# second-state/qwen3_asr_rs

Hardware: AMD Instinct MI355X
Metric: audio-seconds/sec (RTFx) Qwen3-ASR-0.6B greedy, 30s clips (higher is better)
Workload: dtype bf16; 1 GPU; Qwen3-ASR-0.6b bf16, batch=1 x 30s synthetic 16kHz clip per GPU, 100 new tokens (fixed, EOS ignored); clips_per_gpu=1, parallelism=dp1 (independent utterances per GPU, no data-path collective)

## Files before the change

qwen3_asr_rs_amd/csrc/engine.cpp:

```cpp
#include <hip/hip_runtime.h>

#include <sched.h>

#include <chrono>
#include <cmath>
#include <cstdio>
#include <cstring>
#include <map>
#include <memory>
#include <mutex>
#include <thread>

#include "engine_internal.h"

using namespace q3a;

namespace {

thread_local std::string g_last_error;

constexpr int kGemvMaxSeq = 2;

template <typename T>
void upload(DevBuf& b, const std::vector<T>& v, hipStream_t s) {
// ... 73 lines not shown
  const std::vector<hipEvent_t>& join_ev; const hipEvent_t& fork_ev; const int& n_cu; int* const& host_prog_dev;
  std::vector<ProfEvent>* const& prof; Taps& taps;
  const int8_t* const& lm_q; const float* const& lm_qs; const int& lm_q_cols;
  const int &B, &max_ctx, &max_new, &gsize, &live_nsplit_, &attn_nsplit, &min_P_, &part_stride, &beam_w_;
  const size_t& kv_layer_elems; const bool& head_logits_;
  const int &k_parallel_groups, &k_skinny_q, &k_dattn_batched_min_wgs, &k_skinny_glu_hp3, &k_lm_head_prune;
  const bool& logit_bias_on_;
  const bool& sampling_on_;
  const bool& repetition_on_;

  bool precise() const { return opts.precise != 0; }
  bool token_lp() const { return opts.token_logprobs != 0; }
  bool kv_f32() const { return opts.precise != 0; }
  size_t kv_elem() const { return kv_f32() ? 4 : 2; }
  int fast_math() const { return precise() ? 0 : 1; }
  template <typename T> const T* w(uint64_t off) const { return reinterpret_cast<const T*>(arena + off); }
  const float* wf(uint64_t off) const { return w<float>(off); }
  const uint16_t* wh(uint64_t off) const { return w<uint16_t>(off); }
};

struct DecodeStep : StepView {
  DevBuf kcache, vcache, x_dec, d_pos, next_tok, out_ids, step_count, done, s_ln, s_qkv, s_ctx, s_act, logits, part_val, part_idx;
  DevBuf part_sum, out_lp;
  DevBuf blk_lo, blk_hi;
  DevBuf prune_stats;
  DevBuf attn_pm, attn_pl, attn_po, nn_x, nn_ss;
  DevBuf rope_cur, rope_cos, rope_sin;
  DevBuf n_done, forced_tok;
  DevBuf beam_cand_val, beam_cand_idx, beam_part_max, beam_part_sum, beam_topk_ids, beam_topk_lp, beam_score, beam_finished, beam_parent, beam_token;
  DevBuf beam_feed, beam_hist_parent, beam_hist_token, beam_hist_lp, beam_state, beam_lo;
  DevBuf logit_bias;
  DevBuf samp_params, samp_max, samp_sum;
  DevBuf rep_params;
  DevBuf draft_accepted;
  template <class Self, class F> static void each_buf(Self& s, F&& f) {
    for (auto* b : {&s.kcache, &s.vcache, &s.x_dec, &s.d_pos, &s.next_tok, &s.out_ids, &s.step_count, &s.done, &s.s_ln, &s.s_qkv, &s.s_ctx, &s.s_act, &s.logits,
                    &s.part_val, &s.part_idx, &s.part_sum, &s.out_lp, &s.blk_lo, &s.blk_hi, &s.prune_stats, &s.attn_pm, &s.attn_pl, &s.attn_po, &s.nn_x, &s.nn_ss,
                    &s.rope_cur, &s.rope_cos, &s.rope_sin, &s.n_done, &s.forced_tok,
                    &s.beam_cand_val, &s.beam_cand_idx, &s.beam_part_max, &s.beam_part_sum, &s.beam_topk_ids, &s.beam_topk_lp, &s.beam_score, &s.beam_finished,
                    &s.beam_parent, &s.beam_token, &s.beam_feed, &s.beam_hist_parent, &s.beam_hist_token, &s.beam_hist_lp, &s.beam_state, &s.beam_lo,
                    &s.logit_bias, &s.samp_params, &s.samp_max, &s.samp_sum, &s.rep_params, &s.draft_accepted})
      f(*b);
  }

  void tap(const char* name, const void* ptr, size_t bytes) { taps.copy(opts.debug_taps, stream, name, ptr, bytes); }
  template <class F> void timed(int kclass, double bytes, F&& fn) {
    if (!prof) return fn();
    ProfEvent pe{kclass, bytes, nullptr, nullptr};
    HIPCHK(hipEventCreate(&pe.a));
    HIPCHK(hipEventCreate(&pe.b));
    HIPCHK(hipEventRecord(pe.a, stream));
    fn();
    HIPCHK(hipEventRecord(pe.b, stream));
    prof->push_back(pe);
  }

  void* kc_layer(int l) { return (uint8_t*)kcache.p + (size_t)l * kv_layer_elems * kv_elem(); }
  void* vc_layer(int l) { return (uint8_t*)vcache.p + (size_t)l * kv_layer_elems * kv_elem(); }

  LmHeadPruneArgs prune_args(const GemvArgs& g) {
    LmHeadPruneArgs pa{};
    pa.g = g; pa.Wq = lm_q; pa.qcols = lm_q_cols; pa.qs = lm_qs;
    pa.blk_lo = blk_lo.as<float>(); pa.blk_hi = blk_hi.as<float>(); pa.stats = prune_stats.as<int>();
    pa.logit_bias = g.bias != nullptr;
    return pa;
  }

  const float* head_bias() const { return logit_bias_on_ ? logit_bias.as<float>() : nullptr; }

  void run_head(int advance) {
    const int S = B, H = d.hidden, V = d.vocab;
    const float* const hb = head_bias();
    const bool sample = sampling_on_, repeat = repetition_on_, store = head_logits_ || sample || repeat;
    tap("head_in", x_dec.p, (size_t)S * H * 4);
    const double wbytes = 2.0 * V * H;
    int n_part = 0;
    const ArgmaxPartials part{part_val.as<float>(), part_idx.as<int>(), token_lp() ? part_sum.as<float>() : nullptr, part_stride};
    if (S <= kGemvMaxSeq) {
      GemvArgs g{};
      g.fast_math = fast_math();
      g.x = x_dec.as<float>(); g.ldx = H; g.rms_w = wf(L.final_norm); g.eps = d.rms_eps;
      g.W = wh(L.lm_head); g.N = V; g.K = H; g.mode = 3; g.out = logits.as<float>(); g.ldo = V;
      g.part = part; g.bias = hb;
      LmHeadPruneArgs pa{};
      const bool prunable = S == 1 && !precise() && lm_q_cols > 0 && (pa = prune_args(g), !lm_head_prune_check(pa));
      if (prunable && opts.debug_taps == 1) {
        DevBuf& t = taps.reserve("lm_head_bound", (size_t)V * 8);
        LmHeadPruneArgs pd = pa;
        pd.dbg = t.as<float>(); pd.stats = nullptr;
        KCHK(launch_lm_head_approx(pd, stream));
      }
      if (prunable && k_lm_head_prune && !store) {
        g.out = nullptr; pa.g.out = nullptr;
        n_part = lm_head_rescore_groups(g, n_cu);
        timed(Q3A_KC_GEMV_LM_HEAD, (double)V * lm_q_cols, [&] { KCHK(launch_lm_head_approx(pa, stream)); });
        timed(Q3A_KC_ARGMAX, 0, [&] { KCHK(launch_lm_head_rescore(pa, n_part, stream)); });
      } else {
        n_part = gemv_blocks(g);
        timed(Q3A_KC_GEMV_LM_HEAD, wbytes, [&] { KCHK(launch_gemv(g, S, stream)); });
      }
    } else if (!precise()) {
      timed(Q3A_KC_NORM, 0, [&] { KCHK(launch_rmsnorm(x_dec.as<float>(), wf(L.final_norm), s_ln.as<float>(), S, H, d.rms_eps, stream, s_ln.as<uint16_t>())); });
      GemmEpilogue ep; ep.out = logits.as<float>(); ep.ldo = V; ep.bias = hb;
      if (S <= 32 && V % 4 == 0 && H % 64 == 0 && part_stride >= (V + 63) / 64) {
        ep.part = part;
        if (!store) ep.out = nullptr;
        n_part = (V + 63) / 64;
        timed(Q3A_KC_GEMM, wbytes, [&] { KCHK(launch_gemm16(s_ln.as<uint16_t>(), H, wh(L.lm_head), S, V, H, ep, false, stream)); });
      } else {
        timed(Q3A_KC_GEMM, wbytes, [&] { KCHK(launch_gemm16(s_ln.as<uint16_t>(), H, wh(L.lm_head), S, V, H, ep, false, stream)); });
        n_part = 128;
        if (!repeat) timed(Q3A_KC_ARGMAX, 0, [&] { KCHK(launch_argmax_partials(logits.as<float>(), V, S, part, n_part, stream)); });
      }
    } else {
      timed(Q3A_KC_NORM, 0, [&] { KCHK(launch_rmsnorm(x_dec.as<float>(), wf(L.final_norm), s_ln.as<float>(), S, H, d.rms_eps, stream)); });
      timed(Q3A_KC_GEMM, wbytes, [&] { batched_proj(s_ln.as<float>(), H, wh(L.lm_head), V, H, hb, 0, logits.as<float>(), V, nullptr); });
      n_part = 128;
      if (!repeat) timed(Q3A_KC_ARGMAX, 0, [&] { KCHK(launch_argmax_partials(logits.as<float>(), V, S, part, n_part, stream)); });
    }
    if (repeat) n_part = enqueue_repetition(part, !sample);
    FinalizeArgs f{};
    f.part = part; f.n_part = n_part; f.out_lp = part.sum ? out_lp.as<float>() : nullptr;
    f.V = V; f.next_tok = next_tok.as<int>(); f.out_ids = out_ids.as<int>();
    f.out_stride = max_new; f.step_count = step_count.as<int>(); f.pos = d_pos.as<int>(); f.advance = advance;
    f.done = done.as<uint8_t>(); f.n_done = n_done.as<int>(); f.n_seq = S; f.host_progress = host_prog_dev; f.embed = wh(L.embed); f.H = H; f.x_next = x_dec.as<float>(); f.eos0 = kEos0; f.eos1 = kEos1;
    f.cos_t = rope_cos.as<float>(); f.sin_t = rope_sin.as<float>(); f.rope_cur = rope_cur.as<float>();
    f.nn = first_layer_norm_out();
    if (sample) enqueue_sampler(f);
    timed(Q3A_KC_ARGMAX, 0, [&] { KCHK(launch_argmax_finalize(f, S, stream)); });
    if (sample && token_lp()) enqueue_sample_logprob();
  }
  void enqueue_draft_accept(DraftAcceptArgs a) {
    a.n_seq = B; a.accepted = draft_accepted.as<int>();
    a.next_tok = next_tok.as<int>(); a.out_ids = out_ids.as<int>(); a.out_stride = max_new; a.step_count = step_count.as<int>(); a.pos = d_pos.as<int>();
    a.out_lp = token_lp() ? out_lp.as<float>() : nullptr;
    a.done = done.as<uint8_t>(); a.n_done = n_done.as<int>(); a.host_progress = host_prog_dev;
    a.embed = wh(L.embed); a.H = d.hidden; a.x_next = x_dec.as<float>(); a.eos0 = kEos0; a.eos1 = kEos1;
    a.cos_t = rope_cos.as<float>(); a.sin_t = rope_sin.as<float>(); a.rope_cur = rope_cur.as<float>();
    a.nn = first_layer_norm_out();
    timed(Q3A_KC_ARGMAX, 0, [&] { KCHK(launch_draft_accept(a, stream)); });
  }
  int enqueue_repetition(const ArgmaxPartials& part, bool partials) {
    RepeatArgs ra{};
    ra.logits = logits.as<float>(); ra.S = B; ra.V = d.vocab; ra.params = rep_params.as<uint32_t>();
    ra.out_ids = out_ids.as<int>(); ra.out_stride = max_new; ra.step_count = step_count.as<int>();
    timed(Q3A_KC_ARGMAX, 0, [&] { KCHK(launch_repeat_apply(ra, stream)); });
    constexpr int kRepeatParts = 128;
    if (partials) timed(Q3A_KC_ARGMAX, 0, [&] { KCHK(launch_argmax_partials(ra.logits, ra.V, ra.S, part, kRepeatParts, stream)); });
    return kRepeatParts;
  }
// ... 330 lines not shown

  void init_common(const std::string& model_dir, int dev, const q3a_opts* o) {
    if (o) opts = *o; else q3a_opts_default(&opts);
    if (opts.max_new_tokens <= 0) opts.max_new_tokens = 4096;
    d = parse_config_file(model_dir + "/config.json");
    validate_dims(d);
    L = plan_arena(d);
    device = dev;
    int n_dev = 0;
    hipError_t e = hipGetDeviceCount(&n_dev);
    if (e != hipSuccess || n_dev == 0)
      fail("no HIP device available: libq3asr_hip has no CPU fallback (hipGetDeviceCount: " + std::string(hipGetErrorString(e)) + ")");
    if (dev < 0 || dev >= n_dev) fail("device index out of range");
    HIPCHK(hipSetDevice(dev));
    KCHK(skinny_init());
    (void)hipDeviceGetAttribute(&n_cu, hipDeviceAttributeMultiprocessorCount, dev);
    HIPCHK(hipStreamCreateWithFlags(&stream, hipStreamNonBlocking));
    for (auto& x : ev) HIPCHK(hipEventCreate(&x));
    HIPCHK(hipHostMalloc((void**)&host_prog, 64, hipHostMallocMapped));
    memset(host_prog, 0, 64);
    HIPCHK(hipHostGetDevicePointer((void**)&host_prog_dev, host_prog, 0));
    step.n_done.ensure(64);
    step.prune_stats.ensure(8);
    HIPCHK(hipMemsetAsync(step.prune_stats.p, 0, 8, stream));
    if (!d.aligner()) {
      step.logit_bias.ensure((size_t)d.vocab * 4);
      HIPCHK(hipMemsetAsync(step.logit_bias.p, 0, (size_t)d.vocab * 4, stream));
      logit_bias_finite_ = d.vocab;
      step.samp_params.ensure(16);
      step.rep_params.ensure(16);
    }
  }

  void init_tables() {
    auto dftm = make_dft_matrix(400, 416);
    auto filt = make_mel_filterbank_T(d.n_mels, 400, 16000, 202);
    auto pe = make_sinusoid_rows(d.tokens_per_chunk(), d.enc_d);
    upload(dft, dftm, stream);
    upload(filt_t, filt, stream);
    upload(pos_emb, pe, stream);
    zero_page.ensure(256);
    HIPCHK(hipMemsetAsync(zero_page.p, 0, 256, stream));
    ensure_rope(8192);
    HIPCHK(hipStreamSynchronize(stream));
  }

// ... 381 lines not shown
    kv_layer_elems = (size_t)b * d.n_kv * max_ctx * 128;
    step.kcache.ensure(kv_layer_elems * d.dec_layers * kv_elem());
    step.vcache.ensure(kv_layer_elems * d.dec_layers * kv_elem());
    step.rope_cur.ensure((size_t)b * 128 * 4);
    {
      Knobs& kn = knobs();
      const int gs = kn.decode_group_size.load();
      gsize = (gs >= 1 && gs <= 32) ? gs : 32;
      k_parallel_groups = kn.decode_parallel_groups.load(); k_skinny_q = kn.skinny_q.load();
      k_dattn_batched_min_wgs = kn.dattn_batched_min_wgs.load();
      k_skinny_glu_hp3 = kn.skinny_glu_hp3.load();
      k_lm_head_prune = kn.lm_head_prune.load();
    }
    const size_t ng = (size_t)step.n_groups(b);
    step.nn_x.ensure(ng * 32 * H * 2); step.nn_ss.ensure((size_t)ng * (H / 8) * 32 * 4);
    step.x_dec.ensure((size_t)b * H * 4); step.next_tok.ensure((size_t)b * 4); step.forced_tok.ensure((size_t)b * 4); step.draft_accepted.ensure((size_t)b * 8);
    step.out_ids.ensure((size_t)b * max_new * 4); step.step_count.ensure((size_t)b * 4); step.done.ensure((size_t)b);
    step.s_ln.ensure((size_t)b * H * 4); step.s_qkv.ensure((size_t)b * d.qkv_dim() * 4); step.s_ctx.ensure(ng * 32 * d.q_dim() * 4);
    step.s_act.ensure(ng * 32 * d.inter * 4); step.logits.ensure((size_t)b * d.vocab * 4);
    part_stride = std::max(128, (d.vocab + 3) / 4);
    step.part_val.ensure((size_t)b * part_stride * 4); step.part_idx.ensure((size_t)b * part_stride * 4);
    if (token_lp()) { step.part_sum.ensure((size_t)b * part_stride * 4); step.out_lp.ensure((size_t)b * max_new * 4); }
    if (sampling_on_) { step.samp_max.ensure((size_t)b * sample_chunks(d.vocab) * 4); step.samp_sum.ensure((size_t)b * sample_chunks(d.vocab) * 4); }
    {
      const size_t nblk4 = ((size_t)(d.vocab + 15) / 16 + 3) & ~size_t(3);
      step.blk_lo.ensure(nblk4 * 4); step.blk_hi.ensure(nblk4 * 4);
    }
    attn_nsplit = (max_ctx + dattn_keys_per_split(kv_f32()) - 1) / dattn_keys_per_split(kv_f32());
    {
      const size_t n_stat = (size_t)b * d.n_q * attn_nsplit;
      step.attn_pm.ensure((n_stat + 8) * 4); step.attn_pl.ensure((n_stat + 8) * 4);
      step.attn_po.ensure(n_stat * 128 * 4);
      if (knobs().poison_attn_partials.load() != 0) {
        HIPCHK(hipMemsetAsync(step.attn_pm.p, 0xFF, step.attn_pm.cap, stream));
        HIPCHK(hipMemsetAsync(step.attn_pl.p, 0xFF, step.attn_pl.cap, stream));
        HIPCHK(hipMemsetAsync(step.attn_po.p, 0xFF, step.attn_po.cap, stream));
      }
    }
    HIPCHK(hipMemsetAsync(step.step_count.p, 0, (size_t)b * 4, stream));
    HIPCHK(hipMemsetAsync(step.done.p, 0, (size_t)b, stream));
    HIPCHK(hipMemsetAsync(step.n_done.p, 0, 64, stream));
    HIPCHK(hipMemsetAsync(step.out_ids.p, 0, (size_t)b * max_new * 4, stream));
    if (token_lp()) HIPCHK(hipMemsetAsync(step.out_lp.p, 0, (size_t)b * max_new * 4, stream));
    HIPCHK(hipStreamSynchronize(stream));
    for (auto cs : chain_streams) HIPCHK(hipStreamSynchronize(cs));
    __atomic_store_n(&host_prog[0], 0, __ATOMIC_RELAXED);
    __atomic_store_n(&host_prog[1], 0, __ATOMIC_RELAXED);
    drain_retired_graphs();
    {
      bool any = false;
      DecodeStep::each_buf(step, [&](DevBuf& sb) { any = any || sb.grew; sb.grew = false; });
      if (any) drop_graphs();
    }
  }

  void run_prefill() {
    run_prefill_layers();
    const int H = d.hidden;
    KCHK(launch_gather_rows(dec_x.as<float>(), last_rows.as<int>(), B, H, step.x_dec.as<float>(), stream));
    tap("dec_last_hidden", step.x_dec.p, (size_t)B * H * 4);
    step.run_head(0);
    tap("logits", step.logits.p, (size_t)B * d.vocab * 4);
    HIPCHK(hipGetLastError());
    have_prefill = true;
// ... 1415 lines not shown
```

qwen3_asr_rs_amd/csrc/k_decode.hip:

```cpp
#include "argmax.h"
#include "embed_row.h"

namespace q3a {

namespace {

__global__ void embed_kernel(const int* __restrict__ ids, const uint16_t* __restrict__ embed, int H, int skip_id,
                             float* __restrict__ out) {
  const int r = blockIdx.x;
  const int id = ids[r];
  if (id == skip_id) return;
  const uint2* src = reinterpret_cast<const uint2*>(embed + (size_t)id * H);
  float4* dst = reinterpret_cast<float4*>(out + (size_t)r * H);
  for (int i = threadIdx.x; i < H / 4; i += blockDim.x) {
    const uint2 v = src[i];
    dst[i] = make_float4(bf16lo(v.x), bf16hi(v.x), bf16lo(v.y), bf16hi(v.y));
  }
}

__global__ void set_tokens_kernel(const int* __restrict__ tok, const uint16_t* __restrict__ embed, int H,
                                  float* __restrict__ x_next, int* __restrict__ next_tok, NextNormOut nn) {
  __shared__ float red[16];
  const int s = blockIdx.x;
  const int id = tok[s];
// ... 90 lines not shown
  for (int o = 32; o > 0; o >>= 1) m.merge_lane(o);
  if (lane == 0) {
    bv[wave] = m.v; bi[wave] = m.i;
    if constexpr (LP) bs[wave] = m.s;
  }
  __syncthreads();
  if (tid == 0) {
    for (int w = 1; w < 16; ++w) m.merge(bv[w], bi[w], bs[LP ? w : 0]);
    int idx = m.i;
    float lp = 0.f;
    if constexpr (LP) {
      lp = -logf(m.s);
      if (lp > 0.f) lp = 0.f;
    }
    if (idx < 0 || idx >= a.V) { idx = 0; lp = __int_as_float(0x7fc00000); }
    tok_s = idx;
    a.next_tok[s] = idx;
    if (sc < a.out_stride) a.out_ids[(size_t)s * a.out_stride + sc] = idx;
    if constexpr (LP) {
      if (sc < a.out_stride) a.out_lp[(size_t)s * a.out_stride + sc] = lp;
    }
    a.step_count[s] = sc + 1;
    a.pos[s] = np;
    if ((idx == a.eos0 || idx == a.eos1) && !was_done) {
      a.done[s] = 1;
      if (a.n_done) {
        const int n = atomicAdd(a.n_done, 1) + 1;
        if (n == a.n_seq && a.host_progress) __hip_atomic_store(a.host_progress + 1, 1, __ATOMIC_RELAXED, __HIP_MEMORY_SCOPE_SYSTEM);
      }
    }
    if (s == 0 && a.host_progress) __hip_atomic_store(a.host_progress, sc + 1, __ATOMIC_RELAXED, __HIP_MEMORY_SCOPE_SYSTEM);
  }
  __syncthreads();
  if (a.rope_cur && tid < 128) a.rope_cur[(size_t)s * 128 + tid] = rope_v;
  embed_row(a.embed, tok_s, a.H, a.x_next, s, a.nn, bv);
}

}

const char* launch_embed(const int* ids, int rows, const uint16_t* embed, int H, int skip_id, float* out,
                         hipStream_t s) {
  if (rows <= 0) return nullptr;
  hipLaunchKernelGGL(embed_kernel, dim3(rows), dim3(256), 0, s, ids, embed, H, skip_id, out);
  return nullptr;
}
const char* launch_set_tokens(const int* tok, int S, const uint16_t* embed, int H, float* x_next, int* next_tok,
// ... 33 lines not shown
```

qwen3_asr_rs_amd/csrc/k_gemv.hip:

```cpp
#include <algorithm>

#include "argmax.h"


namespace q3a {

int gemv_rows_per_wave(const GemvArgs& a) {
  const int logical = (a.mode == 2) ? a.N / 2 : a.N;
  static const int mid = [] { const char* e = getenv("Q3A_GEMV_PR_MID"); return e ? atoi(e) : 2; }();
  static const int small = [] { const char* e = getenv("Q3A_GEMV_PR_SMALL"); return e ? atoi(e) : 1; }();
  if (logical >= 32768 && a.K <= 2048) return 4;
  if (logical >= 4096 || a.mode == 2) return (mid == 4 || mid == 2) ? mid : 2;
  return (small == 1 || small == 2 || small == 4) ? small : 1;
}
int gemv_blocks(const GemvArgs& a) {
  const int pr = gemv_rows_per_wave(a);
  const int rows_per_wave = (a.mode == 2) ? pr / 2 : pr;
  const int logical = (a.mode == 2) ? a.N / 2 : a.N;
  return (logical + 4 * rows_per_wave - 1) / (4 * rows_per_wave);
}

namespace {

constexpr int ATTN_F_MAX = 1024;
// ... 369 lines not shown
  for (int it = 0; it < KI; ++it)
#pragma unroll
    for (int i = 0; i < PR; ++i) acc[i][0] = dot8(wq[it][i], x[it], acc[i][0]);
  if (wave == 0) asm volatile("" ::"v"(acc[0][0]));
  Q3A_STAMP_AT(a.stamp, blockIdx.x, 3);
  float rstd = 1.0f;
  if (RMS) rstd = rstd_of(wave_sum_fast(ss) / (float)K + a.eps, a.fast_math != 0);
#pragma unroll
  for (int i = 0; i < PR; ++i) acc[i][0] = wave_sum_fast(acc[i][0]) * rstd + bv[i];
  if (lane != 0) return;
  if (a.mode != 2) {
#pragma unroll
    for (int i = 0; i < PR; ++i)
      if (prow[i] >= 0) a.out[prow[i]] = acc[i][0] + rv[i];
  } else {
#pragma unroll
    for (int i = 0; i + 1 < PR; i += 2)
      if (prow[i] >= 0) a.out[g * (PR / 2) + (i >> 1)] = silu_sel(acc[i][0], a.fast_math != 0) * acc[i + 1][0];
  }
  Q3A_STAMP_AT(a.stamp, blockIdx.x, 4);
}

template <int PR, int KI, bool LP = false>
__device__ __forceinline__ void gemv1_head_block(const GemvArgs& a, int blk, float (&am_v)[4][1], int (&am_i)[4][1], float* am_s,
                                                 ArgmaxAcc<LP>& out) {
  const int tid = threadIdx.x, lane = tid & 63, wave = tid >> 6;
  const int K = a.K;
  const int g = blk * 4 + wave;
  int prow[PR];
  gemv_rows<PR>(a, g, prow);
  bool kin[KI];
  int kk[KI];
#pragma unroll
  for (int it = 0; it < KI; ++it) {
    const int k = lane * 8 + it * 512;
    kin[it] = k < K;
    kk[it] = kin[it] ? k : 0;
  }
  float4 xr[KI][2], nr[KI][2];
  uint4 wq[KI][PR];
#pragma unroll
  for (int it = 0; it < KI; ++it) {
    xr[it][0] = *reinterpret_cast<const float4*>(a.x + kk[it]);
    xr[it][1] = *reinterpret_cast<const float4*>(a.x + kk[it] + 4);
    nr[it][0] = *reinterpret_cast<const float4*>(a.rms_w + kk[it]);
    nr[it][1] = *reinterpret_cast<const float4*>(a.rms_w + kk[it] + 4);
  }
#pragma unroll
  for (int it = 0; it < KI; ++it)
#pragma unroll
    for (int i = 0; i < PR; ++i) {
// ... 14 lines not shown
    for (int e = 0; e < 8; ++e) x[it][e] = (K == KI * 512 || kin[it]) ? xv[e] : 0.f;
    const float4 w0 = nr[it][0], w1 = nr[it][1];
    const float wv[8] = {w0.x, w0.y, w0.z, w0.w, w1.x, w1.y, w1.z, w1.w};
#pragma unroll
    for (int e = 0; e < 8; ++e) { ss += x[it][e] * x[it][e]; x[it][e] *= wv[e]; }
  }
  float acc[PR];
#pragma unroll
  for (int i = 0; i < PR; ++i) acc[i] = 0.f;
#pragma unroll
  for (int it = 0; it < KI; ++it)
#pragma unroll
    for (int i = 0; i < PR; ++i) acc[i] = dot8(wq[it][i], x[it], acc[i]);
  const float rstd = rstd_of(wave_sum_fast(ss) / (float)K + a.eps, a.fast_math != 0);
#pragma unroll
  for (int i = 0; i < PR; ++i) acc[i] = wave_sum_fast(acc[i]) * rstd + bv[i];
  ArgmaxAcc<LP> m;
#pragma unroll
  for (int i = 0; i < PR; ++i) {
    if (prow[i] < 0) continue;
    if (lane == 0 && a.out) a.out[prow[i]] = acc[i];
    if (acc[i] > m.v) { m.v = acc[i]; m.i = prow[i]; }
  }
  if (lane == 0) { am_v[wave][0] = m.v; am_i[wave][0] = m.i; }
  if constexpr (LP) {
    float ws = 0.f;
#pragma unroll
    for (int i = 0; i < PR; ++i) ws += prow[i] < 0 ? 0.f : lse_term(1.f, acc[i], m.v);
    if (lane == 0) am_s[wave] = ws;
  }
  __syncthreads();
  if (tid == 0) {
    out = {am_v[0][0], am_i[0][0], LP ? am_s[0] : 0.f};
    for (int w = 1; w < 4; ++w) out.merge(am_v[w][0], am_i[w][0], LP ? am_s[w] : 0.f);
  }
}

template <int PR, int KI, bool LP = false>
__global__ __launch_bounds__(256) void gemv1_head_kernel(GemvArgs a) {
  __shared__ float am_v[4][1];
  __shared__ int am_i[4][1];
  __shared__ float am_s[LP ? 4 : 1];
  ArgmaxAcc<LP> r;
  gemv1_head_block<PR, KI, LP>(a, blockIdx.x, am_v, am_i, am_s, r);
  if (threadIdx.x == 0) r.store(a.part, 0, blockIdx.x);
}

struct LmHeadArgsDev {
  GemvArgs g;
  const int8_t* Wq; const float* qs; int qcols;
  float gamma;
  float* blk_lo; float* blk_hi; int n_blk;
  float* dbg;
  int* stats;
};

__device__ __forceinline__ float dotq8(uint32_t lo, uint32_t hi, const float (&x)[8], float s) {
  f32x2_t a = f32x2_t{(float)(int8_t)lo, (float)(int8_t)(lo >> 8)} * f32x2_t{x[0], x[1]};
  a += f32x2_t{(float)(int8_t)(lo >> 16), (float)((int32_t)lo >> 24)} * f32x2_t{x[2], x[3]};
  a += f32x2_t{(float)(int8_t)hi, (float)(int8_t)(hi >> 8)} * f32x2_t{x[4], x[5]};
  a += f32x2_t{(float)(int8_t)(hi >> 16), (float)((int32_t)hi >> 24)} * f32x2_t{x[6], x[7]};
  return s + (a.x + a.y);
}

__global__ __launch_bounds__(256) void lm_head_quantize_kernel(const uint16_t* W, int N, int K, int cols, int8_t* Q, float* qs) {
  const int lane = threadIdx.x & 63, r = blockIdx.x * 4 + (threadIdx.x >> 6);
  if (r >= N) return;
  const uint16_t* w = W + (size_t)r * K;
  float m = 0.f;
  for (int k = lane; k < K; k += 64) m = fmaxf(m, fabsf(__uint_as_float((uint32_t)w[k] << 16)));
  m = wave_max(m);
  const bool fin = isfinite(m);
  const float s = fin ? (float)((double)m / 127.0) : 0.f;
  double dn = 0.0, wn = 0.0, qn = 0.0;
  for (int k = lane; k < K; k += 64) {
    const double v = __uint_as_float((uint32_t)w[k] << 16);
    const double q = s > 0.f ? fmin(127.0, fmax(-127.0, rint(v / (double)s))) : 0.0;
    Q[(size_t)r * cols + ((k % 512) / 8) * (cols / 64) + (k / 512) * 8 + k % 8] = (int8_t)q;
    const double e = v - (double)s * q;
    dn += e * e; wn += v * v; qn += q * q;
  }
#pragma unroll
  for (int o = 32; o >= 1; o >>= 1) {
    dn += __shfl_xor(dn, o); wn += __shfl_xor(wn, o); qn += __shfl_xor(qn, o);
  }
  if (lane == 0) {
    auto up = [](double v) {
      v *= 1.0 + 0x1p-40;
      const float f = (float)v;
      return (double)f < v ? nextafterf(f, INFINITY) : f;
    };
    float4 o = make_float4(s, up(sqrt(dn)), up(sqrt(wn)), up((double)s * sqrt(qn)));
    if (!fin || !isfinite(o.y) || !isfinite(o.z)) o = make_float4(0.f, INFINITY, INFINITY, 0.f);
    reinterpret_cast<float4*>(qs)[r] = o;
  }
}

template <int KI, bool BIAS>
__device__ __forceinline__ void lm_head_approx_body(const LmHeadArgsDev& p) {
  constexpr int R = 16, NQ = KI / 2;
  const GemvArgs& a = p.g;
  const int lane = threadIdx.x & 63, wave = threadIdx.x >> 6;
  const int K = a.K, blk = blockIdx.x * 4 + wave;
  if (blk >= p.n_blk) return;
  bool kin[KI];
  int kk[KI];
#pragma unroll
  for (int it = 0; it < KI; ++it) {
    const int k = lane * 8 + it * 512;
    kin[it] = k < K;
    kk[it] = kin[it] ? k : 0;
  }
  float4 xr[KI][2], nr[KI][2];
#pragma unroll
  for (int it = 0; it < KI; ++it) {
    xr[it][0] = *reinterpret_cast<const float4*>(a.x + kk[it]);
    xr[it][1] = *reinterpret_cast<const float4*>(a.x + kk[it] + 4);
    nr[it][0] = *reinterpret_cast<const float4*>(a.rms_w + kk[it]);
    nr[it][1] = *reinterpret_cast<const float4*>(a.rms_w + kk[it] + 4);
  }
  uint4 wq[R][NQ];
#pragma unroll
  for (int i = 0; i < R; ++i) {
    const int r = blk * R + i, row = r < a.N ? r : a.N - 1;
#pragma unroll
    for (int j = 0; j < NQ; ++j) wq[i][j] = ld_stream16(p.Wq + (size_t)row * p.qcols + lane * (KI * 8) + j * 16);
  }
// ... 18 lines not shown
#pragma unroll
    for (int e = 0; e < 8; ++e) yy += x[it][e] * x[it][e];
  }
  float acc[R];
#pragma unroll
  for (int i = 0; i < R; ++i) {
    acc[i] = 0.f;
#pragma unroll
    for (int j = 0; j < NQ; ++j) {
      acc[i] = dotq8(wq[i][j].x, wq[i][j].y, x[2 * j], acc[i]);
      acc[i] = dotq8(wq[i][j].z, wq[i][j].w, x[2 * j + 1], acc[i]);
    }
  }
  const float rstd = rstd_of(wave_sum_fast(ss) / (float)K + a.eps, a.fast_math != 0);
  const float ny = sqrtf(wave_sum_fast(yy));
  float mine = 0.f;
#pragma unroll
  for (int i = 0; i < R; ++i) {
    const float t = wave_sum_fast(acc[i]);
    if (lane == i) mine = t;
  }
  const float av = (mine * q.x) * rstd;
  const float ev = (rstd * ny) * (q.y + p.gamma * (q.z + q.w)) * (1.0f + 0x1p-10f) + fabsf(av) * 0x1p-20f + 1e-30f;
  float lo = -INFINITY, hi = -INFINITY;
  if constexpr (BIAS) {
    if (my_valid) {
      const float ab = av + bq;
      const float eb = (ev + 0x1p-22f * (fabsf(av) + fabsf(bq))) * (1.0f + 0x1p-20f);
      if (bq == -INFINITY) {
        if (p.dbg) { p.dbg[(size_t)my_r * 2] = -INFINITY; p.dbg[(size_t)my_r * 2 + 1] = 0.f; }
      } else {
        lo = ab - eb;
        hi = ab + eb;
        if (!(lo <= hi) || hi == INFINITY) { lo = -INFINITY; hi = INFINITY; }
        if (p.dbg) { p.dbg[(size_t)my_r * 2] = ab; p.dbg[(size_t)my_r * 2 + 1] = eb; }
      }
    }
  } else if (my_valid) {
    lo = av - ev;
    hi = av + ev;
    if (!(lo <= hi) || hi == INFINITY) { lo = -INFINITY; hi = INFINITY; }
    if (p.dbg) { p.dbg[(size_t)my_r * 2] = av; p.dbg[(size_t)my_r * 2 + 1] = ev; }
  }
  lo = wave_max(lo);
  hi = wave_max(hi);
  if (lane == 0) { p.blk_lo[blk] = lo; p.blk_hi[blk] = hi; }
}

template <int KI>
__global__ __launch_bounds__(256) void lm_head_approx_kernel(LmHeadArgsDev p) { lm_head_approx_body<KI, false>(p); }
template <int KI>
__global__ __launch_bounds__(256) void lm_head_approx_bias_kernel(LmHeadArgsDev p) { lm_head_approx_body<KI, true>(p); }

template <int PR, int KI>
__global__ __launch_bounds__(256) void lm_head_rescore_kernel(LmHeadArgsDev p) {
  __shared__ float am_v[4][1];
  __shared__ int am_i[4][1];
  __shared__ float red[4];
  __shared__ int cand[256];
  constexpr int PRE = 10;
  const int tid = threadIdx.x, lane = tid & 63, wave = tid >> 6;
  const int nb = p.n_blk, n4 = (nb + 3) / 4, G = gridDim.x;
  const float4* lo4 = reinterpret_cast<const float4*>(p.blk_lo);
  float4 lv[PRE];
#pragma unroll
  for (int j = 0; j < PRE; ++j) {
    const int i4 = tid + j * 256;
    lv[j] = lo4[i4 < n4 ? i4 : n4 - 1];
  }
  const int mb = blockIdx.x + tid * G;
  const float hv = p.blk_hi[mb < nb ? mb : nb - 1];
  float t = -INFINITY;
  auto fold = [&](const float4& v, int i4) {
    const int i = i4 * 4;
    if (i < nb) t = fmaxf(t, v.x);
    if (i + 1 < nb) t = fmaxf(t, v.y);
    if (i + 2 < nb) t = fmaxf(t, v.z);
    if (i + 3 < nb) t = fmaxf(t, v.w);
  };
#pragma unroll
  for (int j = 0; j < PRE; ++j) fold(lv[j], tid + j * 256);
  for (int i4 = tid + PRE * 256; i4 < n4; i4 += 256) fold(lo4[i4], i4);
  t = wave_max(t);
  if (lane == 0) red[wave] = t;
  cand[tid] = 0;
  __syncthreads();
  const float T = fmaxf(fmaxf(red[0], red[1]), fmaxf(red[2], red[3]));
  if (mb < nb) cand[tid] = !(hv < T);
  __syncthreads();
  const int nj = (nb - blockIdx.x + G - 1) / G;
  ArgmaxAcc<false> best;
  int nc = 0;
  for (int j = 0; j < nj; ++j) {
    if (!cand[j]) continue;
    ArgmaxAcc<false> r;
    gemv1_head_block<PR, KI>(p.g, blockIdx.x + j * G, am_v, am_i, nullptr, r);
    if (tid == 0) best.merge(r);
    ++nc;
    __syncthreads();
  }
  if (tid == 0) {
    best.store(p.g.part, 0, blockIdx.x);
    if (p.stats) {
      if (nc) atomicAdd(&p.stats[0], nc);
      if (blockIdx.x == 0) atomicAdd(&p.stats[1], 1);
    }
  }
}

template <int NB, int PR, int PF, bool LP = false>
__global__ __launch_bounds__(256) void gemvn_kernel(GemvArgs a) {
  extern __shared__ __attribute__((aligned(16))) float xs[];
  __shared__ float red[NB][4];
  __shared__ float am_v[4][NB];
  __shared__ int am_i[4][NB];
  __shared__ float am_s[LP ? 4 : 1][NB];
  const int tid = threadIdx.x, lane = tid & 63, wave = tid >> 6;
  const int K = a.K;
  const int g = blockIdx.x * 4 + wave;
  int prow[PR];
  gemv_rows<PR>(a, g, prow);
  uint4 wq[PF][PR];
#pragma unroll
  for (int it = 0; it < PF; ++it) {
// ... 88 lines not shown
    hipLaunchKernelGGL((gemv1_kernel<PR, KI, true, false>), grid, block, 0, s, a);
  } else {
    hipLaunchKernelGGL((gemv1_kernel<PR, KI, false, false>), grid, block, 0, s, a);
  }
}
template <int PR>
void launch1(const GemvArgs& a, hipStream_t s) {
  if (a.K <= 1024) launch1k<PR, 2>(a, s);
  else if (a.K <= 2048) launch1k<PR, 4>(a, s);
  else if constexpr (PR < 4) {
    if (a.K <= 3072) launch1k<PR, 6>(a, s); else launch1k<PR, 12>(a, s);
  }
}
template <int NB, int PR, int PF>
void launchn(const GemvArgs& a, hipStream_t s) {
  if (a.part.sum) hipLaunchKernelGGL((gemvn_kernel<NB, PR, PF, true>), dim3(gemv_blocks(a)), dim3(256), (size_t)NB * a.K * sizeof(float), s, a);
  else hipLaunchKernelGGL((gemvn_kernel<NB, PR, PF>), dim3(gemv_blocks(a)), dim3(256), (size_t)NB * a.K * sizeof(float), s, a);
}

}

static LmHeadArgsDev lm_head_dev_args(const LmHeadPruneArgs& a) {
  LmHeadArgsDev p{};
  p.g = a.g; p.Wq = a.Wq; p.qs = a.qs; p.qcols = a.qcols; p.blk_lo = a.blk_lo; p.blk_hi = a.blk_hi; p.n_blk = lm_head_prune_blocks(a.g);
  p.dbg = a.dbg; p.stats = a.stats;
  const double nu = (double)a.qcols * 0x1p-24;
  p.gamma = (float)(nu / (1.0 - nu)) * (1.0f + 0x1p-20f);
  return p;
}
int lm_head_prune_blocks(const GemvArgs& g) { return (g.N + 15) / 16; }
const char* launch_lm_head_quantize(const uint16_t* W, int N, int K, int8_t* Q, float* qs, hipStream_t s) {
  const int cols = lm_head_q_cols(K);
  if (cols == 0 || K % 8 != 0) return "lm_head_quantize: hidden size beyond the one-sequence GEMV";
  if (hipMemsetAsync(Q, 0, (size_t)N * cols, s) != hipSuccess) return "lm_head_quantize: memset failed";
  hipLaunchKernelGGL(lm_head_quantize_kernel, dim3((N + 3) / 4), dim3(256), 0, s, W, N, K, cols, Q, qs);
  return nullptr;
}
const char* lm_head_prune_check(const LmHeadPruneArgs& a) {
  const GemvArgs& g = a.g;
  if (g.mode != 3 || !g.rms_w || !g.x || g.attn_po) return "lm_head_prune: needs the plain mode-3 GEMV with a fused norm";
  if (g.bias && !a.logit_bias) return "lm_head_prune: the only bias the bound covers is the logit bias (finite or -inf entries)";
  if (g.part.sum) return "lm_head_prune: token log-probabilities need every logit (the full GEMV)";
  if (gemv_rows_per_wave(g) != 4 || gemv_blocks(g) != lm_head_prune_blocks(g)) return "lm_head_prune: the GEMV does not run 16-row blocks here";
  if (g.K % 8 != 0 || a.qcols != lm_head_q_cols(g.K)) return "lm_head_prune: int8 row width does not match the hidden size";
  if (!a.Wq || !a.qs || !a.blk_lo || !a.blk_hi || !g.part.val) return "lm_head_prune: missing buffer";
  if (const char* e = argmax_partials_check(g.part, 1)) return e;
  return nullptr;
}
const char* launch_lm_head_approx(const LmHeadPruneArgs& a, hipStream_t s) {
  if (const char* e = lm_head_prune_check(a)) return e;
  const LmHeadArgsDev p = lm_head_dev_args(a);
  const dim3 grid((p.n_blk + 3) / 4), block(256);
  if (a.g.bias) {
    if (a.qcols == 1024) hipLaunchKernelGGL(lm_head_approx_bias_kernel<2>, grid, block, 0, s, p);
    else hipLaunchKernelGGL(lm_head_approx_bias_kernel<4>, grid, block, 0, s, p);
  } else {
    if (a.qcols == 1024) hipLaunchKernelGGL(lm_head_approx_kernel<2>, grid, block, 0, s, p);
    else hipLaunchKernelGGL(lm_head_approx_kernel<4>, grid, block, 0, s, p);
  }
  return nullptr;
}
int lm_head_rescore_groups(const GemvArgs& g, int n_cu) {
  const int nb = lm_head_prune_blocks(g);
  return std::min(nb, std::max(n_cu > 0 ? n_cu : 256, (nb + 255) / 256));
}
const char* launch_lm_head_rescore(const LmHeadPruneArgs& a, int groups, hipStream_t s) {
  if (const char* e = lm_head_prune_check(a)) return e;
  const LmHeadArgsDev p = lm_head_dev_args(a);
  if (groups < 1 || groups > a.g.part.stride || (p.n_blk + groups - 1) / groups > 256) return "lm_head_prune: bad rescore grid";
  if (a.qcols == 1024) hipLaunchKernelGGL((lm_head_rescore_kernel<4, 2>), dim3(groups), dim3(256), 0, s, p);
  else hipLaunchKernelGGL((lm_head_rescore_kernel<4, 4>), dim3(groups), dim3(256), 0, s, p);
  return nullptr;
}

const char* launch_gemv(const GemvArgs& a0, int NB, hipStream_t s) {
  if (a0.K % 8 != 0) return "gemv: K must be a multiple of 8";
  if (a0.K > 6144) return "gemv: K > 6144 unsupported";
  if (a0.mode == 2 && a0.N % 32 != 0) return "gemv: GLU needs N % 32 == 0";
  if (a0.mode == 3 && !a0.rms_w) return "gemv: mode 3 (the lm_head) needs the fused final norm";
  if (a0.mode == 3 && !a0.part.val) return "gemv: argmax partial buffer missing";
  if (const char* e = argmax_partials_check(a0.part, a0.mode == 3 ? gemv_blocks(a0) : 0)) return e;
  if (a0.part.sum && a0.mode != 3) return "gemv: log-sum partials need mode 3";
  if (a0.attn_po && (a0.K % 128 != 0 || a0.K != a0.attn_heads * 128)) return "gemv: attention-partial input needs K = heads*128";
  if (a0.attn_po && a0.rms_w) return "gemv: attention-partial input cannot be combined with a fused RMSNorm";
  if (a0.attn_po && (NB < 4 ? NB : 4) * a0.attn_heads * a0.attn_nsplit > ATTN_F_MAX) return "gemv: too many attention splits for the LDS scale table";
  const int pr = gemv_rows_per_wave(a0);
  const int nb_cap = (int)((64 * 1024) / ((size_t)a0.K * 4));
  int done = 0;
  while (done < NB) {
    GemvArgs a = a0;
    if (a0.x) a.x = a0.x + (size_t)done * a0.ldx;
    if (a0.out) a.out = a0.out + (size_t)done * a0.ldo;
    if (a0.resid) a.resid = a0.resid + (size_t)done * a0.ldo;
    a.part = a0.part.at(done);
// ... 22 lines not shown
```

qwen3_asr_rs_amd/csrc/kernels.h:

```cpp
#pragma once
#include <hip/hip_runtime.h>
#include <stdint.h>

#include <atomic>

#ifndef Q3A_STAMP_FIELD
#ifdef Q3A_STAMP
#define Q3A_STAMP_FIELD unsigned long long* stamp = nullptr;
#else
#define Q3A_STAMP_FIELD
#endif
#endif

namespace q3a {

struct ArgmaxPartials {
  float* val = nullptr;
  int* idx = nullptr;
  float* sum = nullptr;
  int stride = 0;
  ArgmaxPartials at(size_t rows) const {
    const size_t o = rows * stride;
    return {val ? val + o : nullptr, idx ? idx + o : nullptr, sum ? sum + o : nullptr, stride};
  }
// ... 154 lines not shown
  const float* x; int ldx;
  const float* rms_w;
  float eps;
  const uint16_t* W; int N; int K;
  const float* bias;
  int mode;
  float* out; int ldo;
  const float* resid;
  ArgmaxPartials part;
  const float* attn_pm; const float* attn_pl; const float* attn_po; int attn_nsplit; int attn_heads;
  int attn_fast_exp;
  int fast_math;
  Q3A_STAMP_FIELD
};
const char* launch_gemv(const GemvArgs& a, int NB, hipStream_t s);
constexpr int GEMV_ATTN_MAX_TABLE = 1024;
int gemv_blocks(const GemvArgs& a);
int gemv_rows_per_wave(const GemvArgs& a);

struct LmHeadPruneArgs {
  GemvArgs g;
  const int8_t* Wq; int qcols;
  const float* qs;
  float* blk_lo; float* blk_hi;
  float* dbg;
  int* stats;
  int logit_bias;
};
inline int lm_head_q_cols(int hidden) { return hidden <= 1024 ? 1024 : hidden <= 2048 ? 2048 : 0; }
const char* launch_lm_head_quantize(const uint16_t* W, int N, int K, int8_t* Q, float* qs, hipStream_t s);
int lm_head_prune_blocks(const GemvArgs& g);
int lm_head_rescore_groups(const GemvArgs& g, int n_cu);
const char* lm_head_prune_check(const LmHeadPruneArgs& a);
const char* launch_lm_head_approx(const LmHeadPruneArgs& a, hipStream_t s);
const char* launch_lm_head_rescore(const LmHeadPruneArgs& a, int groups, hipStream_t s);

struct SkinnyArgs {
  const float* x; int ldx; int S;
  const uint16_t* x16;
  int x16_frag;
  int out16_frag;
  const float* rms_w; float eps;
  const uint16_t* W; int N; int K;
  const float* bias;
  int mode;
  float* out; int ldo;
  uint16_t* out16;
  const float* resid;
  const uint16_t* xw16f; const float* ss_parts; int ss_nparts;
  const float* next_w; uint16_t* next_xw16f; float* next_ss;
  int qsplit;
  int qs_halves;
  int glu_hp3;
  int n_cu;
  int fast_math;
  Q3A_STAMP_FIELD
};
struct NextNormOut {
// ... 38 lines not shown
                                hipStream_t s, uint16_t* out16 = nullptr, bool frag = false);

struct FinalizeArgs {
  ArgmaxPartials part;
  int n_part;
  int V;
  int* next_tok;
  int* out_ids;
  int out_stride;
  int* step_count;
  int* pos;
  int advance;
  uint8_t* done;
  int* n_done;
  int n_seq;
  int* host_progress;
  const uint16_t* embed; int H;
  float* x_next;
  int eos0, eos1;
  const float* cos_t; const float* sin_t;
  float* rope_cur;
  NextNormOut nn;
  float* out_lp;
};
const char* launch_argmax_partials(const float* logits, int V, int S, const ArgmaxPartials& p, int nblk, hipStream_t s);
const char* launch_argmax_finalize(const FinalizeArgs& a, int S, hipStream_t s);
const char* launch_set_tokens(const int* tok, int S, const uint16_t* embed, int H, float* x_next, int* next_tok, hipStream_t s,
                              const NextNormOut& nn = NextNormOut{});

struct DraftAcceptArgs {
  int n_seq;
  const int* draft; const int* draft_off;
  const int* prompt_len;
  const int* top_id; const float* top_lp;
  int* accepted;
  int* next_tok; int* out_ids; int out_stride; int* step_count; int* pos;
  float* out_lp;
  uint8_t* done; int* n_done; int* host_progress;
  const uint16_t* embed; int H; float* x_next; int eos0, eos1;
  const float* cos_t; const float* sin_t; float* rope_cur;
  NextNormOut nn;
};
const char* launch_draft_accept(const DraftAcceptArgs& a, hipStream_t s);

constexpr int BEAM_MAX_W = 8;
constexpr int BEAM_CHUNK = 2048;
// ... 64 lines not shown
```

Baseline: 482.7 audio-seconds/sec.

## Fuse LM-head int8 bound pass and exact rescore into one kernel

Replaces the two-kernel pruned LM head (int8 bound pre-pass writing per-block lo/hi arrays, then a rescore kernel that reduces a global threshold) with a single fused kernel. Each workgroup computes bounds for its contiguous block range, keeps hi values in LDS, and publishes its lo floor through a global atomic max that other groups read opportunistically. It then rescores surviving candidate blocks with full bf16 GEMV waves. This removes one launch and the global round trip for the bound arrays. The threshold can be looser because groups may not see each other's floors, so more blocks may be rescored. A floor reset is added to argmax finalize.

```diff
diff --git a/qwen3_asr_rs_amd/csrc/engine.cpp b/qwen3_asr_rs_amd/csrc/engine.cpp
--- a/qwen3_asr_rs_amd/csrc/engine.cpp
+++ b/qwen3_asr_rs_amd/csrc/engine.cpp
@@ -119,7 +119,7 @@
 struct DecodeStep : StepView {
   DevBuf kcache, vcache, x_dec, d_pos, next_tok, out_ids, step_count, done, s_ln, s_qkv, s_ctx, s_act, logits, part_val, part_idx;
   DevBuf part_sum, out_lp;
-  DevBuf blk_lo, blk_hi;
+  DevBuf head_floor;
   DevBuf prune_stats;
   DevBuf attn_pm, attn_pl, attn_po, nn_x, nn_ss;
   DevBuf rope_cur, rope_cos, rope_sin;
@@ -132,7 +132,7 @@
   DevBuf draft_accepted;
   template <class Self, class F> static void each_buf(Self& s, F&& f) {
     for (auto* b : {&s.kcache, &s.vcache, &s.x_dec, &s.d_pos, &s.next_tok, &s.out_ids, &s.step_count, &s.done, &s.s_ln, &s.s_qkv, &s.s_ctx, &s.s_act, &s.logits,
-                    &s.part_val, &s.part_idx, &s.part_sum, &s.out_lp, &s.blk_lo, &s.blk_hi, &s.prune_stats, &s.attn_pm, &s.attn_pl, &s.attn_po, &s.nn_x, &s.nn_ss,
+                    &s.part_val, &s.part_idx, &s.part_sum, &s.out_lp, &s.head_floor, &s.prune_stats, &s.attn_pm, &s.attn_pl, &s.attn_po, &s.nn_x, &s.nn_ss,
                     &s.rope_cur, &s.rope_cos, &s.rope_sin, &s.n_done, &s.forced_tok,
                     &s.beam_cand_val, &s.beam_cand_idx, &s.beam_part_max, &s.beam_part_sum, &s.beam_topk_ids, &s.beam_topk_lp, &s.beam_score, &s.beam_finished,
                     &s.beam_parent, &s.beam_token, &s.beam_feed, &s.beam_hist_parent, &s.beam_hist_token, &s.beam_hist_lp, &s.beam_state, &s.beam_lo,
@@ -158,7 +158,7 @@
   LmHeadPruneArgs prune_args(const GemvArgs& g) {
     LmHeadPruneArgs pa{};
     pa.g = g; pa.Wq = lm_q; pa.qcols = lm_q_cols; pa.qs = lm_qs;
-    pa.blk_lo = blk_lo.as<float>(); pa.blk_hi = blk_hi.as<float>(); pa.stats = prune_stats.as<int>();
+    pa.stats = prune_stats.as<int>(); pa.floor = head_floor.as<int>();
     pa.logit_bias = g.bias != nullptr;
     return pa;
   }
@@ -189,9 +189,8 @@
       }
       if (prunable && k_lm_head_prune && !store) {
         g.out = nullptr; pa.g.out = nullptr;
-        n_part = lm_head_rescore_groups(g, n_cu);
-        timed(Q3A_KC_GEMV_LM_HEAD, (double)V * lm_q_cols, [&] { KCHK(launch_lm_head_approx(pa, stream)); });
-        timed(Q3A_KC_ARGMAX, 0, [&] { KCHK(launch_lm_head_rescore(pa, n_part, stream)); });
+        n_part = lm_head_fused_groups(g, n_cu);
+        timed(Q3A_KC_GEMV_LM_HEAD, (double)V * lm_q_cols, [&] { KCHK(launch_lm_head_fused(pa, n_part, stream)); });
       } else {
         n_part = gemv_blocks(g);
         timed(Q3A_KC_GEMV_LM_HEAD, wbytes, [&] { KCHK(launch_gemv(g, S, stream)); });
@@ -223,6 +222,7 @@
     f.done = done.as<uint8_t>(); f.n_done = n_done.as<int>(); f.n_seq = S; f.host_progress = host_prog_dev; f.embed = wh(L.embed); f.H = H; f.x_next = x_dec.as<float>(); f.eos0 = kEos0; f.eos1 = kEos1;
     f.cos_t = rope_cos.as<float>(); f.sin_t = rope_sin.as<float>(); f.rope_cur = rope_cur.as<float>();
     f.nn = first_layer_norm_out();
+    f.head_floor = head_floor.as<int>();
     if (sample) enqueue_sampler(f);
     timed(Q3A_KC_ARGMAX, 0, [&] { KCHK(launch_argmax_finalize(f, S, stream)); });
     if (sample && token_lp()) enqueue_sample_logprob();
@@ -599,6 +599,8 @@
     HIPCHK(hipHostGetDevicePointer((void**)&host_prog_dev, host_prog, 0));
     step.n_done.ensure(64);
     step.prune_stats.ensure(8);
+    step.head_floor.ensure(4);
+    HIPCHK(hipMemsetD32Async((hipDeviceptr_t)step.head_floor.p, LM_HEAD_FLOOR_NONE, 1, stream));
     HIPCHK(hipMemsetAsync(step.prune_stats.p, 0, 8, stream));
     if (!d.aligner()) {
       step.logit_bias.ensure((size_t)d.vocab * 4);
@@ -1026,10 +1028,6 @@
     step.part_val.ensure((size_t)b * part_stride * 4); step.part_idx.ensure((size_t)b * part_stride * 4);
     if (token_lp()) { step.part_sum.ensure((size_t)b * part_stride * 4); step.out_lp.ensure((size_t)b * max_new * 4); }
     if (sampling_on_) { step.samp_max.ensure((size_t)b * sample_chunks(d.vocab) * 4); step.samp_sum.ensure((size_t)b * sample_chunks(d.vocab) * 4); }
-    {
-      const size_t nblk4 = ((size_t)(d.vocab + 15) / 16 + 3) & ~size_t(3);
-      step.blk_lo.ensure(nblk4 * 4); step.blk_hi.ensure(nblk4 * 4);
-    }
     attn_nsplit = (max_ctx + dattn_keys_per_split(kv_f32()) - 1) / dattn_keys_per_split(kv_f32());
     {
       const size_t n_stat = (size_t)b * d.n_q * attn_nsplit;
@@ -1044,6 +1042,7 @@
     HIPCHK(hipMemsetAsync(step.step_count.p, 0, (size_t)b * 4, stream));
     HIPCHK(hipMemsetAsync(step.done.p, 0, (size_t)b, stream));
     HIPCHK(hipMemsetAsync(step.n_done.p, 0, 64, stream));
+    HIPCHK(hipMemsetD32Async((hipDeviceptr_t)step.head_floor.p, LM_HEAD_FLOOR_NONE, 1, stream));
     HIPCHK(hipMemsetAsync(step.out_ids.p, 0, (size_t)b * max_new * 4, stream));
     if (token_lp()) HIPCHK(hipMemsetAsync(step.out_lp.p, 0, (size_t)b * max_new * 4, stream));
     HIPCHK(hipStreamSynchronize(stream));
diff --git a/qwen3_asr_rs_amd/csrc/k_decode.hip b/qwen3_asr_rs_amd/csrc/k_decode.hip
--- a/qwen3_asr_rs_amd/csrc/k_decode.hip
+++ b/qwen3_asr_rs_amd/csrc/k_decode.hip
@@ -136,6 +136,7 @@
     }
     a.step_count[s] = sc + 1;
     a.pos[s] = np;
+    if (a.head_floor && s == 0) *a.head_floor = LM_HEAD_FLOOR_NONE;
     if ((idx == a.eos0 || idx == a.eos1) && !was_done) {
       a.done[s] = 1;
       if (a.n_done) {
diff --git a/qwen3_asr_rs_amd/csrc/k_gemv.hip b/qwen3_asr_rs_amd/csrc/k_gemv.hip
--- a/qwen3_asr_rs_amd/csrc/k_gemv.hip
+++ b/qwen3_asr_rs_amd/csrc/k_gemv.hip
@@ -415,11 +415,8 @@
 }
 
 template <int PR, int KI, bool LP = false>
-__device__ __forceinline__ void gemv1_head_block(const GemvArgs& a, int blk, float (&am_v)[4][1], int (&am_i)[4][1], float* am_s,
-                                                 ArgmaxAcc<LP>& out) {
-  const int tid = threadIdx.x, lane = tid & 63, wave = tid >> 6;
+__device__ __forceinline__ ArgmaxAcc<LP> gemv1_head_wave(const GemvArgs& a, int g, int lane) {
   const int K = a.K;
-  const int g = blk * 4 + wave;
   int prow[PR];
   gemv_rows<PR>(a, g, prow);
   bool kin[KI];
@@ -480,12 +477,23 @@
     if (lane == 0 && a.out) a.out[prow[i]] = acc[i];
     if (acc[i] > m.v) { m.v = acc[i]; m.i = prow[i]; }
   }
-  if (lane == 0) { am_v[wave][0] = m.v; am_i[wave][0] = m.i; }
   if constexpr (LP) {
     float ws = 0.f;
 #pragma unroll
     for (int i = 0; i < PR; ++i) ws += prow[i] < 0 ? 0.f : lse_term(1.f, acc[i], m.v);
-    if (lane == 0) am_s[wave] = ws;
+    m.s = ws;
+  }
+  return m;
+}
+
+template <int PR, int KI, bool LP = false>
+__device__ __forceinline__ void gemv1_head_block(const GemvArgs& a, int blk, float (&am_v)[4][1], int (&am_i)[4][1], float* am_s,
+                                                 ArgmaxAcc<LP>& out) {
+  const int tid = threadIdx.x, lane = tid & 63, wave = tid >> 6;
+  const ArgmaxAcc<LP> m = gemv1_head_wave<PR, KI, LP>(a, blk * 4 + wave, lane);
+  if (lane == 0) {
+    am_v[wave][0] = m.v; am_i[wave][0] = m.i;
+    if constexpr (LP) am_s[wave] = m.s;
   }
   __syncthreads();
   if (tid == 0) {
@@ -508,9 +516,10 @@
   GemvArgs g;
   const int8_t* Wq; const float* qs; int qcols;
   float gamma;
-  float* blk_lo; float* blk_hi; int n_blk;
+  int n_blk;
   float* dbg;
   int* stats;
+  int* floor;
 };
 
 __device__ __forceinline__ float dotq8(uint32_t lo, uint32_t hi, const float (&x)[8], float s) {
@@ -555,12 +564,10 @@
 }
 
 template <int KI, bool BIAS>
-__device__ __forceinline__ void lm_head_approx_body(const LmHeadArgsDev& p) {
+__device__ __forceinline__ void lm_head_block_bounds(const LmHeadArgsDev& p, int blk, int lane, float& lo, float& hi) {
   constexpr int R = 16, NQ = KI / 2;
   const GemvArgs& a = p.g;
-  const int lane = threadIdx.x & 63, wave = threadIdx.x >> 6;
-  const int K = a.K, blk = blockIdx.x * 4 + wave;
-  if (blk >= p.n_blk) return;
+  const int K = a.K;
   bool kin[KI];
   int kk[KI];
 #pragma unroll
@@ -625,7 +632,7 @@
   }
   const float av = (mine * q.x) * rstd;
   const float ev = (rstd * ny) * (q.y + p.gamma * (q.z + q.w)) * (1.0f + 0x1p-10f) + fabsf(av) * 0x1p-20f + 1e-30f;
-  float lo = -INFINITY, hi = -INFINITY;
+  lo = -INFINITY; hi = -INFINITY;
   if constexpr (BIAS) {
     if (my_valid) {
       const float ab = av + bq;
@@ -647,62 +654,64 @@
   }
   lo = wave_max(lo);
   hi = wave_max(hi);
-  if (lane == 0) { p.blk_lo[blk] = lo; p.blk_hi[blk] = hi; }
-}
-
+}
+
+template <int KI, bool BIAS>
+__device__ __forceinline__ void lm_head_approx_body(const LmHeadArgsDev& p) {
+  const int blk = blockIdx.x * 4 + (threadIdx.x >> 6);
+  if (blk >= p.n_blk) return;
+  float lo, hi;
+  lm_head_block_bounds<KI, BIAS>(p, blk, threadIdx.x & 63, lo, hi);
+}
 template <int KI>
 __global__ __launch_bounds__(256) void lm_head_approx_kernel(LmHeadArgsDev p) { lm_head_approx_body<KI, false>(p); }
 template <int KI>
 __global__ __launch_bounds__(256) void lm_head_approx_bias_kernel(LmHeadArgsDev p) { lm_head_approx_body<KI, true>(p); }
 
-template <int PR, int KI>
-__global__ __launch_bounds__(256) void lm_head_rescore_kernel(LmHeadArgsDev p) {
-  __shared__ float am_v[4][1];
-  __shared__ int am_i[4][1];
-  __shared__ float red[4];
-  __shared__ int cand[256];
-  constexpr int PRE = 10;
-  const int tid = threadIdx.x, lane = tid & 63, wave = tid >> 6;
-  const int nb = p.n_blk, n4 = (nb + 3) / 4, G = gridDim.x;
-  const float4* lo4 = reinterpret_cast<const float4*>(p.blk_lo);
-  float4 lv[PRE];
-#pragma unroll
-  for (int j = 0; j < PRE; ++j) {
-    const int i4 = tid + j * 256;
-    lv[j] = lo4[i4 < n4 ? i4 : n4 - 1];
-  }
-  const int mb = blockIdx.x + tid * G;
-  const float hv = p.blk_hi[mb < nb ? mb : nb - 1];
-  float t = -INFINITY;
-  auto fold = [&](const float4& v, int i4) {
-    const int i = i4 * 4;
-    if (i < nb) t = fmaxf(t, v.x);
-    if (i + 1 < nb) t = fmaxf(t, v.y);
-    if (i + 2 < nb) t = fmaxf(t, v.z);
-    if (i + 3 < nb) t = fmaxf(t, v.w);
-  };
-#pragma unroll
-  for (int j = 0; j < PRE; ++j) fold(lv[j], tid + j * 256);
-  for (int i4 = tid + PRE * 256; i4 < n4; i4 += 256) fold(lo4[i4], i4);
-  t = wave_max(t);
-  if (lane == 0) red[wave] = t;
-  cand[tid] = 0;
+constexpr int LM_HEAD_RUN_MAX = 1024;
+__device__ __forceinline__ int float_key(float f) { const int b = __float_as_int(f); return b >= 0 ? b : b ^ 0x7fffffff; }
+__device__ __forceinline__ float key_float(int k) { return __int_as_float(k >= 0 ? k : k ^ 0x7fffffff); }
+template <int KI, bool BIAS>
+__global__ __launch_bounds__(KI == 2 ? 1024 : 512) void lm_head_fused_kernel(LmHeadArgsDev p) {
+  constexpr int NW = KI == 2 ? 16 : 8;
+  __shared__ float hi_s[LM_HEAD_RUN_MAX];
+  __shared__ int t_s;
+  __shared__ float bv[NW];
+  __shared__ int bi[NW];
+  const int lane = threadIdx.x & 63, wave = __builtin_amdgcn_readfirstlane(threadIdx.x >> 6);
+  const int b0 = (int)((long long)blockIdx.x * p.n_blk / gridDim.x);
+  const int n = (int)((long long)(blockIdx.x + 1) * p.n_blk / gridDim.x) - b0;
+  if (threadIdx.x == 0) t_s = LM_HEAD_FLOOR_NONE;
   __syncthreads();
-  const float T = fmaxf(fmaxf(red[0], red[1]), fmaxf(red[2], red[3]));
-  if (mb < nb) cand[tid] = !(hv < T);
+  for (int j = wave; j < n; j += NW) {
+    float lo, hi;
+    lm_head_block_bounds<KI, BIAS>(p, b0 + j, lane, lo, hi);
+    if (lane == 0) {
+      hi_s[j] = hi;
+      const int k = float_key(lo);
+      if (atomicMax(&t_s, k) < k) __hip_atomic_fetch_max(p.floor, k, __ATOMIC_RELAXED, __HIP_MEMORY_SCOPE_AGENT);
+    }
+  }
   __syncthreads();
-  const int nj = (nb - blockIdx.x + G - 1) / G;
+  int tk = t_s;
+  tk = max(tk, __hip_atomic_load(p.floor, __ATOMIC_RELAXED, __HIP_MEMORY_SCOPE_AGENT));
+  const float T = key_float(tk);
   ArgmaxAcc<false> best;
   int nc = 0;
-  for (int j = 0; j < nj; ++j) {
-    if (!cand[j]) continue;
-    ArgmaxAcc<false> r;
-    gemv1_head_block<PR, KI>(p.g, blockIdx.x + j * G, am_v, am_i, nullptr, r);
-    if (tid == 0) best.merge(r);
-    ++nc;
-    __syncthreads();
-  }
-  if (tid == 0) {
+  for (int j0 = 0; j0 < n; j0 += 64) {
+    const float h = j0 + lane < n ? hi_s[j0 + lane] : -INFINITY;
+    unsigned long long cand = __ballot(h > -INFINITY && !(h < T));
+    while (cand) {
+      const int j = j0 + __builtin_ctzll(cand);
+      cand &= cand - 1;
+      if (nc % (NW / 4) == (wave >> 2)) best.merge(gemv1_head_wave<4, KI>(p.g, (b0 + j) * 4 + (wave & 3), lane));
+      ++nc;
+    }
+  }
+  if (lane == 0) { bv[wave] = best.v; bi[wave] = best.i; }
+  __syncthreads();
+  if (wave == 0 && lane == 0) {
+    for (int w = 1; w < NW; ++w) best.merge(bv[w], bi[w], 0.f);
     best.store(p.g.part, 0, blockIdx.x);
     if (p.stats) {
       if (nc) atomicAdd(&p.stats[0], nc);
@@ -837,8 +846,8 @@
 
 static LmHeadArgsDev lm_head_dev_args(const LmHeadPruneArgs& a) {
   LmHeadArgsDev p{};
-  p.g = a.g; p.Wq = a.Wq; p.qs = a.qs; p.qcols = a.qcols; p.blk_lo = a.blk_lo; p.blk_hi = a.blk_hi; p.n_blk = lm_head_prune_blocks(a.g);
-  p.dbg = a.dbg; p.stats = a.stats;
+  p.g = a.g; p.Wq = a.Wq; p.qs = a.qs; p.qcols = a.qcols; p.n_blk = lm_head_prune_blocks(a.g);
+  p.dbg = a.dbg; p.stats = a.stats; p.floor = a.floor;
   const double nu = (double)a.qcols * 0x1p-24;
   p.gamma = (float)(nu / (1.0 - nu)) * (1.0f + 0x1p-20f);
   return p;
@@ -858,12 +867,13 @@
   if (g.part.sum) return "lm_head_prune: token log-probabilities need every logit (the full GEMV)";
   if (gemv_rows_per_wave(g) != 4 || gemv_blocks(g) != lm_head_prune_blocks(g)) return "lm_head_prune: the GEMV does not run 16-row blocks here";
   if (g.K % 8 != 0 || a.qcols != lm_head_q_cols(g.K)) return "lm_head_prune: int8 row width does not match the hidden size";
-  if (!a.Wq || !a.qs || !a.blk_lo || !a.blk_hi || !g.part.val) return "lm_head_prune: missing buffer";
+  if (!a.Wq || !a.qs || !g.part.val) return "lm_head_prune: missing buffer";
   if (const char* e = argmax_partials_check(g.part, 1)) return e;
   return nullptr;
 }
 const char* launch_lm_head_approx(const LmHeadPruneArgs& a, hipStream_t s) {
   if (const char* e = lm_head_prune_check(a)) return e;
+  if (!a.dbg) return "lm_head_prune: the pre-pass alone only fills the debug tap";
   const LmHeadArgsDev p = lm_head_dev_args(a);
   const dim3 grid((p.n_blk + 3) / 4), block(256);
   if (a.g.bias) {
@@ -875,16 +885,22 @@
   }
   return nullptr;
 }
-int lm_head_rescore_groups(const GemvArgs& g, int n_cu) {
+int lm_head_fused_groups(const GemvArgs& g, int n_cu) {
   const int nb = lm_head_prune_blocks(g);
-  return std::min(nb, std::max(n_cu > 0 ? n_cu : 256, (nb + 255) / 256));
-}
-const char* launch_lm_head_rescore(const LmHeadPruneArgs& a, int groups, hipStream_t s) {
+  return std::min(nb, std::max(n_cu > 0 ? n_cu : 256, (nb + LM_HEAD_RUN_MAX - 1) / LM_HEAD_RUN_MAX));
+}
+const char* launch_lm_head_fused(const LmHeadPruneArgs& a, int groups, hipStream_t s) {
   if (const char* e = lm_head_prune_check(a)) return e;
   const LmHeadArgsDev p = lm_head_dev_args(a);
-  if (groups < 1 || groups > a.g.part.stride || (p.n_blk + groups - 1) / groups > 256) return "lm_head_prune: bad rescore grid";
-  if (a.qcols == 1024) hipLaunchKernelGGL((lm_head_rescore_kernel<4, 2>), dim3(groups), dim3(256), 0, s, p);
-  else hipLaunchKernelGGL((lm_head_rescore_kernel<4, 4>), dim3(groups), dim3(256), 0, s, p);
+  if (groups < 1 || groups > p.n_blk || groups > a.g.part.stride || (p.n_blk + groups - 1) / groups > LM_HEAD_RUN_MAX) return "lm_head_prune: bad grid";
+  if (!a.floor) return "lm_head_prune: missing buffer";
+  if (a.g.bias) {
+    if (a.qcols == 1024) hipLaunchKernelGGL((lm_head_fused_kernel<2, true>), dim3(groups), dim3(1024), 0, s, p);
+    else hipLaunchKernelGGL((lm_head_fused_kernel<4, true>), dim3(groups), dim3(512), 0, s, p);
+  } else {
+    if (a.qcols == 1024) hipLaunchKernelGGL((lm_head_fused_kernel<2, false>), dim3(groups), dim3(1024), 0, s, p);
+    else hipLaunchKernelGGL((lm_head_fused_kernel<4, false>), dim3(groups), dim3(512), 0, s, p);
+  }
   return nullptr;
 }
 
diff --git a/qwen3_asr_rs_amd/csrc/kernels.h b/qwen3_asr_rs_amd/csrc/kernels.h
--- a/qwen3_asr_rs_amd/csrc/kernels.h
+++ b/qwen3_asr_rs_amd/csrc/kernels.h
@@ -200,18 +200,19 @@
   GemvArgs g;
   const int8_t* Wq; int qcols;
   const float* qs;
-  float* blk_lo; float* blk_hi;
   float* dbg;
   int* stats;
+  int* floor;
   int logit_bias;
 };
+constexpr int LM_HEAD_FLOOR_NONE = (int)0x80000000;
 inline int lm_head_q_cols(int hidden) { return hidden <= 1024 ? 1024 : hidden <= 2048 ? 2048 : 0; }
 const char* launch_lm_head_quantize(const uint16_t* W, int N, int K, int8_t* Q, float* qs, hipStream_t s);
 int lm_head_prune_blocks(const GemvArgs& g);
-int lm_head_rescore_groups(const GemvArgs& g, int n_cu);
+int lm_head_fused_groups(const GemvArgs& g, int n_cu);
 const char* lm_head_prune_check(const LmHeadPruneArgs& a);
 const char* launch_lm_head_approx(const LmHeadPruneArgs& a, hipStream_t s);
-const char* launch_lm_head_rescore(const LmHeadPruneArgs& a, int groups, hipStream_t s);
+const char* launch_lm_head_fused(const LmHeadPruneArgs& a, int groups, hipStream_t s);
 
 struct SkinnyArgs {
   const float* x; int ldx; int S;
@@ -296,6 +297,7 @@
   float* rope_cur;
   NextNormOut nn;
   float* out_lp;
+  int* head_floor;
 };
 const char* launch_argmax_partials(const float* logits, int V, int S, const ArgmaxPartials& p, int nblk, hipStream_t s);
 const char* launch_argmax_finalize(const FinalizeArgs& a, int S, hipStream_t s);
```

Result: no change. 478.0 audio-seconds/sec (-1.0%).
